# lisqzqng/Video-based-gait-analysis-for-dementia

Measured on AMD Instinct MI355X. Metric: frames/sec (224x224, seq=16), higher is better.
Workload: dtype f32

## Files before the change

### video-based-gait-analysis-for-dementia_amd/csrc/conv_wino4.hip

```cpp
#include "kernels.h"

#include <cstdio>
#include <cstdlib>

namespace grk {

typedef float f32x4 __attribute__((ext_vector_type(4)));
#define GRNET_LDS_AS __attribute__((address_space(3)))

namespace {

#ifdef GRNET_ABLATION
__device__ unsigned long long g_w4phase[8];
#define W4_TICK(var) const unsigned long long var = __builtin_readcyclecounter()
#else
#define W4_TICK(var) do { } while (0)
#endif

constexpr int kCK = 8;
constexpr int kRaw = 6 * 56;
constexpr int kV = 36 * kCK * 16;
constexpr int kMrow = 20;
constexpr size_t kLdsB = sizeof(float) * (2 * kCK * kRaw + 2 * kV);
static_assert(sizeof(float) * 36 * 16 * kMrow <= kLdsB, "the epilogue tile reuses the staging area");

template <typename T>
__device__ __forceinline__ void landed(T& x) { asm volatile("" : "+v"(x)); }

__device__ __forceinline__ void bt_lo(const float* d, float& r0, float& r1, float& r2) {
    const float t1 = fmaf(-4.f, d[2], d[4]), t2 = fmaf(-4.f, d[1], d[3]);
    r0 = fmaf(4.f, d[0], fmaf(-5.f, d[2], d[4]));
    r1 = t1 + t2;
    r2 = t1 - t2;
}
__device__ __forceinline__ void bt_hi(const float* d, float& r3, float& r4, float& r5) {
    const float u1 = d[4] - d[2], u2 = 2.f * (d[3] - d[1]);
    r3 = u1 + u2;
    r4 = u1 - u2;
    r5 = fmaf(4.f, d[1], fmaf(-5.f, d[3], d[5]));
}

template <int NB, int WD, int ABL, bool WSPLIT>
__device__ __forceinline__ void conv_wino4_body(const ConvArgs& a) {
    constexpr bool PAIR = NB == 2 && !WSPLIT;
    constexpr int NLD = PAIR ? 9 : 18;
    constexpr int TPR = WD / 4, TRG = 14 / TPR, kRawW = (4 * TRG + 2) * WD, UPC = kRawW / 4;
    static_assert(WD == 56 || WD == 28, "tile geometry");
    extern __shared__ __align__(16) float smem[];
    float* raw = smem;
    float* V = raw + 2 * kCK * kRaw;
    const int tid = threadIdx.x, lane = tid & 63, wave = tid >> 6, l15 = lane & 15, lq = lane >> 4;

    const int id = a.blk0 + (WSPLIT ? (int)(blockIdx.x >> 1) : (int)blockIdx.x), nb0 = WSPLIT ? 2 * (int)(blockIdx.x & 1) : 0;
    int bx, by;
    if (a.xcd) {
        const int j = id >> 3, x = id & 7, q = j / a.gy;
        by = j - q * a.gy;
        bx = x * (a.gx >> 3) + q;
    } else {
        bx = id / a.gy;
        by = id - bx * a.gy;
    }
    const int groups = ((a.H >> 2) + TRG - 1) / TRG;
    const int img = bx / groups, r = bx - img * groups;
    const int co0 = WSPLIT ? by * 64 : by * (NB * 16);
    constexpr int cstr = WSPLIT ? 4 : NB;
    if (a.prio == 1) __builtin_amdgcn_s_setprio(1);
    else if (a.prio >= 2) __builtin_amdgcn_s_setprio(3);
    const int HW = a.H * a.W;
    const float* inb = a.in + ((size_t)img * a.in_ctot + a.in_coff) * HW;
    const int g0 = (4 * TRG * r - 1) * WD;

    const __amdgpu_buffer_rsrc_t u_rsrc = __builtin_amdgcn_make_buffer_rsrc((void*)a.w, (short)0, 36 * a.CinPad * a.CoutPad * 4, 0x00020000);
    const __amdgpu_buffer_rsrc_t r_rsrc = __builtin_amdgcn_make_buffer_rsrc((void*)inb, (short)0, a.Cin * HW * 4, 0x00020000);
    typedef float bfrag __attribute__((ext_vector_type(PAIR ? 4 : NB)));
    const int nchunks_u = a.CinPad / kCK;
    const int ub = PAIR ? ((lq * a.CoutPad * 2 + co0 * 2 + l15 * 4) * 4 + wave * 9 * nchunks_u * 4 * a.CoutPad * 2 * 4)
                        : ((wave * 9 * a.CinPad + lq) * a.CoutPad + co0 + l15 * cstr + nb0) * 4;
    const int u_point = PAIR ? nchunks_u * 4 * a.CoutPad * 2 * 4 : a.CinPad * a.CoutPad * 4;
    const int u_kstep = 4 * a.CoutPad * 4, u_chunk = PAIR ? 4 * a.CoutPad * 2 * 4 : kCK * a.CoutPad * 4;
    auto load_u = [&](int chunk, int g) -> bfrag {
        const int soff = PAIR ? chunk * u_chunk + g * u_point : chunk * u_chunk + (g >> 1) * u_point + (g & 1) * u_kstep;
        if constexpr (PAIR || NB == 4) return __builtin_bit_cast(bfrag, __builtin_amdgcn_raw_buffer_load_b128(u_rsrc, ub, soff, 0));
        else return __builtin_bit_cast(bfrag, __builtin_amdgcn_raw_buffer_load_b64(u_rsrc, ub, soff, 0));
    };
    int roff[3];
#pragma unroll
    for (int i = 0; i < 3; ++i) {
        const int u = i * 256 + tid, ch = u / UPC, k = u - ch * UPC, gi = g0 + 4 * k;
        const bool unit = u < kCK * UPC, inside = gi >= 0 && gi < HW;
        roff[i] = unit && inside ? (ch * HW + gi) * 4 : -1;
        if (unit && !inside) {
            *reinterpret_cast<f32x4*>(raw + u * 4) = f32x4{0.f, 0.f, 0.f, 0.f};
            *reinterpret_cast<f32x4*>(raw + kCK * kRawW + u * 4) = f32x4{0.f, 0.f, 0.f, 0.f};
        }
    }
    auto issue_raw = [&](int chunk) {
        const int soff = chunk * (kCK * 4) * HW;
        float* dst = raw + (chunk & 1) * (kCK * kRawW);
#pragma unroll
        for (int i = 0; i < 3; ++i)
            if (roff[i] >= 0) __builtin_amdgcn_raw_ptr_buffer_load_lds(r_rsrc, (GRNET_LDS_AS void*)(dst + (i * 256 + wave * 64) * 4), 16, roff[i], soff, 0, 0);
        asm volatile("" ::: "memory");
    };

    const int row16 = tid >> 4, px = tid & 15, chn = row16 & 7;
    const int half = __builtin_amdgcn_readfirstlane(row16 >> 3);
    const int pc = WD == 56 ? px : (px & 7), trl = WD == 56 ? 0 : (px >> 3);
    const bool real = pc < TPR;
    const int rpos = chn * kRawW + (4 * trl) * WD + 4 * (real ? pc : TPR - 1);
    const int slot = real ? trl * TPR + pc : 14 + (WD == 56 ? px - 14 : trl);
    const int vpos = (half * 18) * (kCK * 16) + chn * 16 + slot;
    struct Tf { float d[6][6]; float e[3][6]; };
    auto tf_read = [&](Tf& t, const float* rp) {
#pragma unroll
        for (int i = 0; i < 6; ++i) {
            const f32x4 v = *reinterpret_cast<const f32x4*>(rp + i * WD);
            t.d[i][1] = v[0]; t.d[i][2] = v[1]; t.d[i][3] = v[2]; t.d[i][4] = v[3];
        }
    };
    auto tf_halo = [&](Tf& t) {
#pragma unroll
        for (int i = 0; i < 6; ++i) {
            t.d[i][0] = __int_as_float(__builtin_amdgcn_update_dpp(0, __float_as_int(WD == 56 || real ? t.d[i][4] : 0.f), 0x111, 0xf, 0xf, true));
            t.d[i][5] = __int_as_float(__builtin_amdgcn_update_dpp(0, __float_as_int(real ? t.d[i][1] : 0.f), 0x101, 0xf, 0xf, true));
        }
    };
    auto tf_rows = [&](Tf& t) {
#pragma unroll
        for (int j = 0; j < 6; ++j) {
            const float col[6] = {t.d[0][j], t.d[1][j], t.d[2][j], t.d[3][j], t.d[4][j], t.d[5][j]};
            if (half == 0) bt_lo(col, t.e[0][j], t.e[1][j], t.e[2][j]);
            else bt_hi(col, t.e[0][j], t.e[1][j], t.e[2][j]);
        }
    };
    auto tf_cols = [&](Tf& t, float* vp) {
#pragma unroll
        for (int rr = 0; rr < 3; ++rr) {
            float o[6];
            bt_lo(t.e[rr], o[0], o[1], o[2]);
            bt_hi(t.e[rr], o[3], o[4], o[5]);
#pragma unroll
            for (int c = 0; c < 6; ++c) vp[(rr * 6 + c) * (kCK * 16)] = o[c];
        }
    };

    f32x4 acc[9][NB];
#pragma unroll
    for (int p = 0; p < 9; ++p)
#pragma unroll
        for (int n = 0; n < NB; ++n) acc[p][n] = f32x4{0.f, 0.f, 0.f, 0.f};

    const int nchunks = a.CinPad / kCK;
    bfrag bq[NLD];
    W4_TICK(t_start);
    issue_raw(0);
    if (nchunks > 1) issue_raw(1);
#pragma unroll
    for (int g = 0; g < NLD; ++g) bq[g] = load_u(0, g);
    if constexpr (PAIR) asm volatile("s_waitcnt vmcnt(9)" ::: "memory");
    else asm volatile("s_waitcnt vmcnt(18)" ::: "memory");
    __syncthreads();
    W4_TICK(t_first);
    {
        Tf t;
        tf_read(t, raw + rpos);
        tf_halo(t);
        tf_rows(t);
        tf_cols(t, V + vpos);
    }
    W4_TICK(t_tf0);
    float av[2][6];
    auto load_a = [&](int buf, int c, int set) {
#pragma unroll
        for (int k = 0; k < 6; ++k) {
            const int p = wave * 9 + 3 * c + (k >> 1), ks = k & 1;
            av[set][k] = V[buf * kV + p * (kCK * 16) + (ks * 4 + lq) * 16 + l15];
        }
    };
    auto chunk = [&](int buf, bool with_transform, int next) {
        Tf t;
        const float* rp = raw + (next & 1) * (kCK * kRawW) + rpos;
        float* vp = V + (next & 1) * kV + vpos;
        if (ABL != 3) load_a(buf, 0, 0);
        if (with_transform && ABL != 1 && next + 1 < nchunks) issue_raw(next + 1);
#pragma unroll
        for (int c = 0; c < 3; ++c) {
#pragma unroll
            for (int k = 0; k < 6; ++k) landed(av[c & 1][k]);
            if (with_transform && ABL != 2) {
                if (c == 1) { tf_halo(t); tf_rows(t); }
                if (c == 2) tf_cols(t, vp);
            }
            __builtin_amdgcn_sched_barrier(0);
            if (c < 2 && ABL != 3) load_a(buf, c + 1, (c + 1) & 1);
            if (with_transform && ABL != 1 && c > 0) {
#pragma unroll
                for (int k = 0; k < NLD / 3; ++k) bq[(NLD / 3) * (c - 1) + k] = load_u(next, (NLD / 3) * (c - 1) + k);
            }
            if (with_transform && ABL != 2 && c == 0) tf_read(t, rp);
            __builtin_amdgcn_sched_barrier(0);
#pragma unroll
            for (int k = 0; k < 6; ++k)
#pragma unroll
                for (int n = 0; n < NB; ++n) {
                    const int pi = 3 * c + (k >> 1);
                    const float bfr = PAIR ? bq[pi][(k & 1) * 2 + n] : bq[6 * c + k][n];
                    acc[pi][n] = __builtin_amdgcn_mfma_f32_16x16x4f32(av[c & 1][k], bfr, acc[pi][n], 0, 0, 0);
                }
            __builtin_amdgcn_sched_barrier(0);
        }
        if (with_transform && ABL != 1) {
#pragma unroll
            for (int k = 0; k < NLD / 3; ++k) bq[2 * (NLD / 3) + k] = load_u(next, 2 * (NLD / 3) + k);
        }
    };
    auto meet = [&](bool last) {
        if (last) asm volatile("s_waitcnt vmcnt(0)" ::: "memory");
        else if constexpr (PAIR) asm volatile("s_waitcnt vmcnt(9)" ::: "memory");
        else asm volatile("s_waitcnt vmcnt(18)" ::: "memory");
        __syncthreads();
    };
    for (int ch = 0; ch + 1 < nchunks; ++ch) {
        meet(false);
        chunk(ch & 1, true, ch + 1);
    }
    const bool has_add = a.n_add == 1;
    meet(nchunks > 1);
    const int ec = tid / 14, et = tid - ec * 14, etro = et / TPR, etx = et - etro * TPR, eorow = 4 * (TRG * r + etro);
    const bool ethread = tid < 14 * 16 && eorow < a.H;
    f32x4 radd[4] = {f32x4{0.f, 0.f, 0.f, 0.f}, f32x4{0.f, 0.f, 0.f, 0.f}, f32x4{0.f, 0.f, 0.f, 0.f}, f32x4{0.f, 0.f, 0.f, 0.f}};
    auto fetch_res = [&](int nt) {
        const int co = co0 + (nb0 + nt) * 16 + ec;
        if (has_add && ethread && co < a.Cout) {
            const float* ap = a.add[0] + ((size_t)img * a.add_ctot[0] + a.add_coff[0] + co) * HW + eorow * WD + 4 * etx;
#pragma unroll
            for (int i = 0; i < 4; ++i) radd[i] = *reinterpret_cast<const f32x4*>(ap + i * WD);
        }
    };
    fetch_res(0);
    chunk((nchunks - 1) & 1, false, 0);

    W4_TICK(t_loop);
    float* Mx = smem;
    for (int nt = 0; nt < NB; ++nt) {
        __syncthreads();
#pragma unroll
        for (int pi = 0; pi < 9; ++pi) {
            f32x4 v;
            if constexpr (NB == 4) v = nt == 0 ? acc[pi][0] : nt == 1 ? acc[pi][1] : nt == 2 ? acc[pi][2] : acc[pi][3];
            else v = nt == 0 ? acc[pi][0] : acc[pi][1];
            *reinterpret_cast<f32x4*>(Mx + ((wave * 9 + pi) * 16 + l15) * kMrow + lq * 4) = v;
        }
        __syncthreads();
        const f32x4 rcur[4] = {radd[0], radd[1], radd[2], radd[3]};
        if (nt + 1 < NB) fetch_res(nt + 1);
        if (ethread) {
            const int c = ec, t = et, tx = etx;
            const int co = co0 + (nb0 + nt) * 16 + c, orow = eorow;
            if (co < a.Cout) {
                float s[4][6];
#pragma unroll
                for (int j = 0; j < 6; ++j) {
                    float m[6];
#pragma unroll
                    for (int i = 0; i < 6; ++i) m[i] = Mx[((i * 6 + j) * 16 + c) * kMrow + t];
                    const float p12 = m[1] + m[2], m12 = m[1] - m[2], p34 = m[3] + m[4], m34 = m[3] - m[4];
                    s[0][j] = m[0] + p12 + p34;
                    s[1][j] = fmaf(2.f, m34, m12);
                    s[2][j] = fmaf(4.f, p34, p12);
                    s[3][j] = fmaf(8.f, m34, m12) + m[5];
                }
                const float b = a.bias[co];
                const size_t obase = ((size_t)img * a.out_ctot + a.out_coff + co) * HW + orow * WD + 4 * tx;
#pragma unroll
                for (int i = 0; i < 4; ++i) {
                    const float* q = s[i];
                    const float p12 = q[1] + q[2], m12 = q[1] - q[2], p34 = q[3] + q[4], m34 = q[3] - q[4];
                    f32x4 y = f32x4{q[0] + p12 + p34 + b, fmaf(2.f, m34, m12) + b, fmaf(4.f, p34, p12) + b, fmaf(8.f, m34, m12) + q[5] + b};
                    if (has_add) y += rcur[i];
                    if (a.relu) { y[0] = fmaxf(y[0], 0.f); y[1] = fmaxf(y[1], 0.f); y[2] = fmaxf(y[2], 0.f); y[3] = fmaxf(y[3], 0.f); }
                    *reinterpret_cast<f32x4*>(a.out + obase + i * WD) = y;
                }
            }
        }
    }
#ifdef GRNET_ABLATION
    if ((a.dbg & 8) && tid == 0) {
        W4_TICK(t_end);
        atomicAdd(&g_w4phase[0], t_first - t_start); atomicAdd(&g_w4phase[1], t_tf0 - t_first); atomicAdd(&g_w4phase[2], t_loop - t_tf0);
        atomicAdd(&g_w4phase[3], t_end - t_loop); atomicAdd(&g_w4phase[4], 1ull);
    }
#endif
}

template <int NB, int WD = 56, int ABL = 0, bool WSPLIT = false>
__global__ __launch_bounds__(256) void conv_wino4_f32(const ConvArgs a) { conv_wino4_body<NB, WD, ABL, WSPLIT>(a); }

constexpr int kCKW = 16;
constexpr int kVW = 36 * kCKW * 16;
constexpr size_t kLdsW = sizeof(float) * (2 * kCKW * kRaw + 2 * kVW);
static_assert(sizeof(float) * 2 * 36 * 16 * kMrow <= kLdsW, "the epilogue tiles reuse the staging area");

template <int WD, int NPW>
__device__ __forceinline__ void conv_wino4w_body(const ConvArgs& a) {
    constexpr int TPR = WD / 4, TRG = 14 / TPR, kRawW = (4 * TRG + 2) * WD, UPC = kRawW / 4;
    constexpr int COUTW = 2 * NPW * 16;
    static_assert((WD == 56 || WD == 28) && (NPW == 4 || NPW == 2), "geometry");
    typedef float bfrag __attribute__((ext_vector_type(NPW)));
    extern __shared__ __align__(16) float smem[];
    float* raw = smem;
    float* V = raw + 2 * kCKW * kRaw;
    const int tid = threadIdx.x, lane = tid & 63, wave = __builtin_amdgcn_readfirstlane(tid >> 6), l15 = lane & 15, lq = lane >> 4;
    const int pg = wave & 3, hf = wave >> 2;

    const int id = blockIdx.x;
    int bx, by;
    if (a.xcd) {
        const int j = id >> 3, x = id & 7, q = j / a.gy;
        by = j - q * a.gy;
        bx = x * (a.gx >> 3) + q;
    } else {
        bx = id / a.gy;
        by = id - bx * a.gy;
    }
    const int groups = ((a.H >> 2) + TRG - 1) / TRG;
    const int img = bx / groups, r = bx - img * groups;
    const int co0 = by * COUTW + hf * (NPW * 16);
    const int wpos = NPW == 4 ? co0 : (co0 & ~63) + ((co0 >> 5) & 1) * 2;
    if (a.prio == 1) __builtin_amdgcn_s_setprio(1);
    else if (a.prio >= 2) __builtin_amdgcn_s_setprio(3);
    const int HW = a.H * a.W;
    const float* inb = a.in + ((size_t)img * a.in_ctot + a.in_coff) * HW;
    const int g0 = (4 * TRG * r - 1) * WD;

    const __amdgpu_buffer_rsrc_t u_rsrc = __builtin_amdgcn_make_buffer_rsrc((void*)a.w, (short)0, 36 * a.CinPad * a.CoutPad * 4, 0x00020000);
    const __amdgpu_buffer_rsrc_t r_rsrc = __builtin_amdgcn_make_buffer_rsrc((void*)inb, (short)0, a.Cin * HW * 4, 0x00020000);
    const int ub = ((pg * 9 * a.CinPad + lq) * a.CoutPad + wpos + l15 * 4) * 4;
    const int u_point = a.CinPad * a.CoutPad * 4, u_kstep = 4 * a.CoutPad * 4, u_chunk = kCKW * a.CoutPad * 4;
    auto load_u = [&](int chunk, int q, int e) -> bfrag {
        const int soff = chunk * u_chunk + (3 * (q >> 1) + (e >> 1)) * u_point + (2 * (q & 1) + (e & 1)) * u_kstep;
        if constexpr (NPW == 4) return __builtin_bit_cast(bfrag, __builtin_amdgcn_raw_buffer_load_b128(u_rsrc, ub, soff, 0));
        else return __builtin_bit_cast(bfrag, __builtin_amdgcn_raw_buffer_load_b64(u_rsrc, ub, soff, 0));
    };
    constexpr int NRU = (kCKW * UPC + 511) / 512;
    int roff[NRU];
#pragma unroll
    for (int i = 0; i < NRU; ++i) {
        const int u = i * 512 + tid, ch = u / UPC, k = u - ch * UPC, gi = g0 + 4 * k;
        const bool unit = u < kCKW * UPC, inside = gi >= 0 && gi < HW;
        roff[i] = unit && inside ? (ch * HW + gi) * 4 : -1;
        if (unit && !inside) {
            *reinterpret_cast<f32x4*>(raw + u * 4) = f32x4{0.f, 0.f, 0.f, 0.f};
            *reinterpret_cast<f32x4*>(raw + kCKW * kRawW + u * 4) = f32x4{0.f, 0.f, 0.f, 0.f};
        }
    }
    auto issue_raw = [&](int chunk) {
        const int soff = chunk * (kCKW * 4) * HW;
        float* dst = raw + (chunk & 1) * (kCKW * kRawW);
#pragma unroll
        for (int i = 0; i < NRU; ++i)
            if (roff[i] >= 0) __builtin_amdgcn_raw_ptr_buffer_load_lds(r_rsrc, (GRNET_LDS_AS void*)(dst + (i * 512 + wave * 64) * 4), 16, roff[i], soff, 0, 0);
        asm volatile("" ::: "memory");
    };

    const int row16 = tid >> 4, px = tid & 15, chn = row16 & 15;
    const int pc = WD == 56 ? px : (px & 7), trl = WD == 56 ? 0 : (px >> 3);
    const bool real = pc < TPR;
    const int rpos = chn * kRawW + (4 * trl) * WD + 4 * (real ? pc : TPR - 1);
    const int slot = real ? trl * TPR + pc : 14 + (WD == 56 ? px - 14 : trl);
    const int vpos = (hf * 18) * (kCKW * 16) + chn * 16 + slot;
    auto transform = [&](const float* rp, float* vp) {
        float e[3][6];
        float d[6][6];
#pragma unroll
        for (int i = 0; i < 6; ++i) {
            const f32x4 v = *reinterpret_cast<const f32x4*>(rp + i * WD);
            d[i][1] = v[0]; d[i][2] = v[1]; d[i][3] = v[2]; d[i][4] = v[3];
        }
#pragma unroll
        for (int i = 0; i < 6; ++i) {
            d[i][0] = __int_as_float(__builtin_amdgcn_update_dpp(0, __float_as_int(WD == 56 || real ? d[i][4] : 0.f), 0x111, 0xf, 0xf, true));
            d[i][5] = __int_as_float(__builtin_amdgcn_update_dpp(0, __float_as_int(real ? d[i][1] : 0.f), 0x101, 0xf, 0xf, true));
        }
#pragma unroll
        for (int j = 0; j < 6; ++j) {
            const float col[6] = {d[0][j], d[1][j], d[2][j], d[3][j], d[4][j], d[5][j]};
            if (hf == 0) bt_lo(col, e[0][j], e[1][j], e[2][j]);
            else bt_hi(col, e[0][j], e[1][j], e[2][j]);
        }
#pragma unroll
        for (int rr = 0; rr < 3; ++rr) {
            float o[6];
            bt_lo(e[rr], o[0], o[1], o[2]);
            bt_hi(e[rr], o[3], o[4], o[5]);
#pragma unroll
            for (int c = 0; c < 6; ++c) vp[(rr * 6 + c) * (kCKW * 16)] = o[c];
        }
    };

    f32x4 acc[9][NPW];
#pragma unroll
    for (int p = 0; p < 9; ++p)
#pragma unroll
        for (int n = 0; n < NPW; ++n) acc[p][n] = f32x4{0.f, 0.f, 0.f, 0.f};

    const int nchunks = a.CinPad / kCKW;
    bfrag bq[6];
    float av[2][6];
    auto load_a = [&](int buf, int q, int set) {
#pragma unroll
        for (int e = 0; e < 6; ++e) {
            const int p = pg * 9 + 3 * (q >> 1) + (e >> 1), ks = 2 * (q & 1) + (e & 1);
            av[set][e] = V[buf * kVW + p * (kCKW * 16) + (ks * 4 + lq) * 16 + l15];
        }
    };
    auto multiply = [&](int buf, int ch, bool more) {
        load_a(buf, 0, 0);
#pragma unroll
        for (int q = 0; q < 6; ++q) {
#pragma unroll
            for (int e = 0; e < 6; ++e) landed(av[q & 1][e]);
            __builtin_amdgcn_sched_barrier(0);
            if (q < 5) load_a(buf, q + 1, (q + 1) & 1);
            __builtin_amdgcn_sched_barrier(0);
#pragma unroll
            for (int e = 0; e < 6; ++e) {
                const int pi = 3 * (q >> 1) + (e >> 1);
#pragma unroll
                for (int n = 0; n < NPW; ++n) acc[pi][n] = __builtin_amdgcn_mfma_f32_16x16x4f32(av[q & 1][e], bq[e][n], acc[pi][n], 0, 0, 0);
                __builtin_amdgcn_sched_barrier(0);
                if (q < 5) bq[e] = load_u(ch, q + 1, e);
                else if (more) bq[e] = load_u(ch + 1, 0, e);
                __builtin_amdgcn_sched_barrier(0);
            }
        }
    };

    const bool has_add = a.n_add == 1;
    const int eh = tid >> 8, et2 = tid & 255, ec = et2 / 14, et = et2 - ec * 14, etro = et / TPR, etx = et - etro * TPR, eorow = 4 * (TRG * r + etro);
    const bool ethread = et2 < 14 * 16 && eorow < a.H;
    f32x4 radd[4] = {f32x4{0.f, 0.f, 0.f, 0.f}, f32x4{0.f, 0.f, 0.f, 0.f}, f32x4{0.f, 0.f, 0.f, 0.f}, f32x4{0.f, 0.f, 0.f, 0.f}};
    auto fetch_res = [&](int nt) {
        const int co = by * COUTW + eh * (NPW * 16) + nt * 16 + ec;
        if (has_add && ethread && co < a.Cout) {
            const float* ap = a.add[0] + ((size_t)img * a.add_ctot[0] + a.add_coff[0] + co) * HW + eorow * WD + 4 * etx;
#pragma unroll
            for (int i = 0; i < 4; ++i) radd[i] = *reinterpret_cast<const f32x4*>(ap + i * WD);
        }
    };

    issue_raw(0);
    if (nchunks > 1) issue_raw(1);
#pragma unroll
    for (int e = 0; e < 6; ++e) bq[e] = load_u(0, 0, e);
    asm volatile("s_waitcnt vmcnt(6)" ::: "memory");
    __syncthreads();
    if (hf == 0) transform(raw + rpos, V + vpos);
    for (int k = 0; k < nchunks; ++k) {
        if (hf == 0) {
            asm volatile("s_waitcnt vmcnt(6)" ::: "memory");
            __syncthreads();
            if (k + 2 < nchunks) issue_raw(k + 2);
        }
        const int tk = k + 1 - hf;
        if (tk < nchunks) transform(raw + (tk & 1) * (kCKW * kRawW) + rpos, V + (tk & 1) * kVW + vpos);
        if (hf != 0) {
            asm volatile("s_waitcnt vmcnt(6)" ::: "memory");
            __syncthreads();
            if (k + 2 < nchunks) issue_raw(k + 2);
        }
        if (k + 1 == nchunks) fetch_res(0);
        __builtin_amdgcn_sched_barrier(0);
        multiply(k & 1, k, k + 1 < nchunks);
        __builtin_amdgcn_sched_barrier(0);
    }

    float* Mx = smem + hf * (36 * 16 * kMrow);
    const float* Mr = smem + eh * (36 * 16 * kMrow);
    for (int nt = 0; nt < NPW; ++nt) {
        __syncthreads();
#pragma unroll
        for (int pi = 0; pi < 9; ++pi) {
            f32x4 v;
            if constexpr (NPW == 4) v = nt == 0 ? acc[pi][0] : nt == 1 ? acc[pi][1] : nt == 2 ? acc[pi][2] : acc[pi][3];
            else v = nt == 0 ? acc[pi][0] : acc[pi][1];
            *reinterpret_cast<f32x4*>(Mx + ((pg * 9 + pi) * 16 + l15) * kMrow + lq * 4) = v;
        }
        __syncthreads();
        const f32x4 rcur[4] = {radd[0], radd[1], radd[2], radd[3]};
        if (nt + 1 < NPW) fetch_res(nt + 1);
        if (ethread) {
            const int co = by * COUTW + eh * (NPW * 16) + nt * 16 + ec;
            if (co < a.Cout) {
                float s4[4][6];
#pragma unroll
                for (int j = 0; j < 6; ++j) {
                    float m[6];
#pragma unroll
                    for (int i = 0; i < 6; ++i) m[i] = Mr[((i * 6 + j) * 16 + ec) * kMrow + et];
                    const float p12 = m[1] + m[2], m12 = m[1] - m[2], p34 = m[3] + m[4], m34 = m[3] - m[4];
                    s4[0][j] = m[0] + p12 + p34;
                    s4[1][j] = fmaf(2.f, m34, m12);
                    s4[2][j] = fmaf(4.f, p34, p12);
                    s4[3][j] = fmaf(8.f, m34, m12) + m[5];
                }
                const float b = a.bias[co];
                const size_t obase = ((size_t)img * a.out_ctot + a.out_coff + co) * HW + eorow * WD + 4 * etx;
#pragma unroll
                for (int i = 0; i < 4; ++i) {
                    const float* q = s4[i];
                    const float p12 = q[1] + q[2], m12 = q[1] - q[2], p34 = q[3] + q[4], m34 = q[3] - q[4];
                    f32x4 y = f32x4{q[0] + p12 + p34 + b, fmaf(2.f, m34, m12) + b, fmaf(4.f, p34, p12) + b, fmaf(8.f, m34, m12) + q[5] + b};
                    if (has_add) y += rcur[i];
                    if (a.relu) { y[0] = fmaxf(y[0], 0.f); y[1] = fmaxf(y[1], 0.f); y[2] = fmaxf(y[2], 0.f); y[3] = fmaxf(y[3], 0.f); }
                    *reinterpret_cast<f32x4*>(a.out + obase + i * WD) = y;
                }
            }
        }
    }
}

template <int WD, int NPW>
__global__ __launch_bounds__(512) void conv_wino4w_f32(const ConvArgs a) { conv_wino4w_body<WD, NPW>(a); }

}

int conv_wino4_wide(int cout, int w) {
    static const int wide_env = GRNET_AB(WINO_WIDE, 1);
    if (w == 56) return cout % 128 == 0 ? ((wide_env & 1) ? 4 : 0) : cout == 64 ? ((wide_env & 8) ? 2 : 0) : 0;
    if (w == 28) return cout % 128 == 0 ? ((wide_env & 4) ? 4 : 0) : cout == 64 ? ((wide_env & 2) ? 2 : 0) : 0;
    return 0;
}
int conv_wino4_blocks(int cout, int w) { return (cout % 64 == 0 && !(w == 28 && cout == 64 && !conv_wino4_wide(cout, w))) ? 4 : 2; }

bool conv_wino4_eligible(int cin, int cout, int ks, int stride, int h, int w, int n_add) {
    return ks == 3 && stride == 1 && ((h == 56 && w == 56) || (h == 28 && w == 28)) && n_add <= 1 && cin % kCK == 0 && cout % 32 == 0 && cin >= 32;
}

static size_t wino4_lds() {
    static const size_t pad = (size_t)GRNET_AB(WINO_LDS_PAD, 0);
    return kLdsB + pad;
}

hipError_t conv_wino4_form(const ConvArgs& a, Wino4Form* f) {
    *f = Wino4Form{};
    f->nb = conv_wino4_blocks(a.Cout, a.W);
    if (!conv_wino4_eligible(a.Cin, a.Cout, a.ks, a.stride, a.H, a.W, a.n_add) || a.CinPad % kCK != 0 || a.CoutPad % (f->nb * 16) != 0) return hipErrorInvalidValue;
    if (a.n_add == 1 && a.add_shift[0] != 0) return hipErrorInvalidValue;
    const int npw = conv_wino4_wide(a.Cout, a.W);
    if (npw && a.CinPad % kCKW == 0 && a.CoutPad % (npw * 32) == 0 && !(a.dbg & 32)) {
        const int trg = a.W == 56 ? 1 : 2;
        f->waves = 8;
        f->npw = npw;
        f->gx = a.N * (((a.H >> 2) + trg - 1) / trg);
        f->gy = a.CoutPad / (npw * 32);
        f->xcd = f->gx % 8 == 0 && f->gx >= 16 ? 1 : 0;
        f->full = f->gx * f->gy;
        return hipSuccess;
    }
    const int trg = 14 / (a.W / 4);
    f->waves = 4;
    f->gx = a.N * (((a.H >> 2) + trg - 1) / trg);
    f->gy = a.CoutPad / (f->nb * 16);
    f->xcd = f->gx % 8 == 0 && f->gx >= 16 ? 1 : 0;
    const int total = f->gx * f->gy;
    f->full = total;
    if (f->nb == 2) return hipSuccess;
    static const int split_env = GRNET_AB(WINO_SPLIT, 1);
    int kCUs = 0;
    if (hipError_t e = device_cu_count(&kCUs); e != hipSuccess) return e;
    const int full = total / kCUs * kCUs, rest = total - full;
    if (split_env && full > 0 && rest > 0 && 2 * rest <= kCUs && (!f->xcd || full % 8 == 0)) {
        f->split = 1;
        f->full = full;
        f->rest = rest;
    }
    return hipSuccess;
}

template <int WD>
static hipError_t launch_wino4_w(ConvArgs a, hipStream_t s, const Wino4Form& f, int* n_launches) {
    const size_t kLdsB = wino4_lds();
    a.gx = f.gx;
    a.gy = f.gy;
    a.xcd = f.xcd;
    a.blk0 = 0;
    a.wsplit = 0;
    if (n_launches) *n_launches = 1;
    const int total = a.gx * a.gy;
#ifdef GRNET_ABLATION
    if constexpr (WD == 56) {
        if (a.dbg >= 1 && a.dbg <= 3) {
            auto go = [&](auto kern) { (void)hipFuncSetAttribute(reinterpret_cast<const void*>(kern), hipFuncAttributeMaxDynamicSharedMemorySize, (int)kLdsB); return launch_k(kern, dim3(total), dim3(256), kLdsB, s, a); };
            if (a.dbg == 1) return go(conv_wino4_f32<4, 56, 1>);
            if (a.dbg == 2) return go(conv_wino4_f32<4, 56, 2>);
            return go(conv_wino4_f32<4, 56, 3>);
        }
    }
#endif
    if (f.nb == 2) return launch_k(conv_wino4_f32<2, WD>, dim3(total), dim3(256), kLdsB, s, a);
    if (f.split) {
        hipError_t e = launch_k(conv_wino4_f32<4, WD>, dim3(f.full), dim3(256), kLdsB, s, a);
        if (e != hipSuccess) return e;
        a.blk0 = f.full;
        a.wsplit = 1;
        if (n_launches) *n_launches = 2;
        return launch_k(conv_wino4_f32<2, WD, 0, true>, dim3(2 * f.rest), dim3(256), kLdsB, s, a);
    }
    return launch_k(conv_wino4_f32<4, WD>, dim3(total), dim3(256), kLdsB, s, a);
}

hipError_t launch_conv_wino4(ConvArgs a, hipStream_t s, int* n_launches) {
    static PerDeviceOnce attr;
    int dev = 0;
    if (hipError_t e = current_device(&dev); e != hipSuccess) return e;
    if (hipError_t e = once_per_device(attr, dev, [](int*) {
            hipError_t e = hipSuccess;
            auto set = [&](auto kern) { if (e == hipSuccess) e = hipFuncSetAttribute(reinterpret_cast<const void*>(kern), hipFuncAttributeMaxDynamicSharedMemorySize, (int)wino4_lds()); };
            set(conv_wino4_f32<4, 56>); set(conv_wino4_f32<2, 56>); set(conv_wino4_f32<4, 28>); set(conv_wino4_f32<2, 28>);
            set(conv_wino4_f32<2, 56, 0, true>); set(conv_wino4_f32<2, 28, 0, true>);
            auto setw = [&](auto kern) { if (e == hipSuccess) e = hipFuncSetAttribute(reinterpret_cast<const void*>(kern), hipFuncAttributeMaxDynamicSharedMemorySize, (int)kLdsW); };
            setw(conv_wino4w_f32<56, 4>); setw(conv_wino4w_f32<56, 2>); setw(conv_wino4w_f32<28, 4>); setw(conv_wino4w_f32<28, 2>);
            return e;
        }); e != hipSuccess) return e;
    Wino4Form f;
    if (hipError_t e = conv_wino4_form(a, &f); e != hipSuccess) return e;
    if (f.waves == 8) {
        a.gx = f.gx;
        a.gy = f.gy;
        a.xcd = f.xcd;
        a.blk0 = 0;
        a.wsplit = 0;
        if (n_launches) *n_launches = 1;
        const dim3 grid(a.gx * a.gy);
        if (a.W == 56) return f.npw == 4 ? launch_k(conv_wino4w_f32<56, 4>, grid, dim3(512), kLdsW, s, a) : launch_k(conv_wino4w_f32<56, 2>, grid, dim3(512), kLdsW, s, a);
        return f.npw == 4 ? launch_k(conv_wino4w_f32<28, 4>, grid, dim3(512), kLdsW, s, a) : launch_k(conv_wino4w_f32<28, 2>, grid, dim3(512), kLdsW, s, a);
    }
#ifdef GRNET_ABLATION
    if (GRNET_AB_SET(W4_PHASES)) {
        a.dbg |= 8;
        const hipError_t e = a.W == 56 ? launch_wino4_w<56>(a, s, f, n_launches) : launch_wino4_w<28>(a, s, f, n_launches);
        unsigned long long h[8] = {}, z[8] = {};
        hipStreamSynchronize(s);
        hipMemcpyFromSymbol(h, HIP_SYMBOL(g_w4phase), sizeof(h));
        hipMemcpyToSymbol(HIP_SYMBOL(g_w4phase), z, sizeof(z));
        const double n = h[4] ? (double)h[4] : 1.0;
        fprintf(stderr, "[wino4 phases] %d->%d @%d N%d add %d nb %d wgs %llu: per WG ticks  prologue %.0f  first transform %.0f  chunk loop %.0f (%d chunks)  epilogue %.0f\n",
                a.Cin, a.Cout, a.W, a.N, a.n_add, f.nb, h[4], h[0] / n, h[1] / n, h[2] / n, a.CinPad / kCK, h[3] / n);
        return e;
    }
#endif
    return a.W == 56 ? launch_wino4_w<56>(a, s, f, n_launches) : launch_wino4_w<28>(a, s, f, n_launches);
}

void wino4_transform_filter(const double* g, double* u) {
// ... 36 lines not shown
```

### video-based-gait-analysis-for-dementia_amd/csrc/grnet.cpp

```cpp
#include "../../include/grnet_hip.h"

#include <hip/hip_runtime.h>

#include <cmath>
#include <cstdio>
#include <cstdlib>
#include <algorithm>
#include <cstring>
#include <map>
#include <memory>
#include <string>
#include <tuple>
#include <unordered_map>
#include <vector>

#include "kernels.h"

using namespace grk;

namespace grk { thread_local GraphRecorder* g_recorder = nullptr; }

namespace {

constexpr double kBnEps = 1e-5;
// ... 1084 lines not shown
                } else if (!pinned) {
                    const int pref = from >= 0 ? lane_of[from] : 0;
                    lane = pref;
                    start = std::max(ready, lane_free[pref]);
                    for (int l = 0; l < n_lanes; ++l) {
                        const double st = std::max(ready, lane_free[l]);
                        if (st + hop_us < start) { start = st; lane = l; }
                    }
                }
                if (best < 0 || start < best_start - 1e-9 || (start < best_start + 1e-9 && blevel[i] > blevel[best])) {
                    best = i; best_lane = lane; best_start = start;
                }
            }
            done[best] = 1;
            lane_of[best] = best_lane;
            finish[best] = best_start + est[best];
            lane_free[best_lane] = finish[best];
            for (int u : users[best]) --pending[u];
            order.push_back(best);
        }
        std::vector<Op> out;
        out.reserve(m);
        for (int i : order) {
            Op op = list[i];
            op.lane = lane_of[i];
            op.waits.clear();
            op.record = false;
            out.push_back(std::move(op));
        }
        if (getenv("GRNET_TRACE")) fprintf(stderr, "[grnet] lane schedule: %d ops, estimated makespan %.0f us (sum of estimates %.0f us)\n", m,
                                           *std::max_element(lane_free, lane_free + kLanes), [&] { double t = 0; for (double e : est) t += e; return t; }());
        list.swap(out);
    }

    void analyze_dependencies(std::vector<Op>& ops, std::vector<hipEvent_t>& op_events) {
        std::map<int, std::vector<int>> writers;
        for (int i = 0; i < (int)ops.size(); ++i) {
            Op& op = ops[i];
            for (int buf : op.rd) {
                auto it = writers.find(buf);
                if (it == writers.end()) continue;
                for (int w : it->second)
                    if (ops[w].lane != op.lane) {
                        bool dup = false;
                        for (int x : op.waits) dup |= x == w;
                        if (!dup) op.waits.push_back(w);
                        ops[w].record = true;
                    }
            }
            for (int out : op.wr) writers[out].push_back(i);
        }
        op_events.assign(ops.size(), nullptr);
        if (getenv("GRNET_TRACE")) {
            size_t waits = 0, records = 0;
            for (const Op& op : ops) { waits += op.waits.size(); records += op.record; }
            fprintf(stderr, "[grnet] dependencies: %zu ops, %zu cross-lane waits, %zu recorded events\n", ops.size(), waits, records);
        }
    }

    const HostTensor* find(const std::string& k) const {
        auto it = tensors.find(k);
        return it == tensors.end() ? nullptr : &it->second;
    }

    int upload(const std::vector<float>& h, float** d) {
        int rc = dev_alloc(d, h.size());
        if (rc) return rc;
        if (hipMemcpy(*d, h.data(), h.size() * sizeof(float), hipMemcpyHostToDevice) != hipSuccess)
            return fail(GRNET_EHIP, "hipMemcpy H2D failed");
        return 0;
    }

    int pack_conv(ConvLayer& L) {
        const int cin = L.cin_w, ks = L.ks, taps = ks * ks;
        const int TC = conv_pick_tc(L.cout);
        const bool bf = dtype == 1;
        L.cin_pad = bf ? (L.in.c + L.in2.c + 31) / 32 * 32 : (cin + kConvCK - 1) / kConvCK * kConvCK;
        if (L.in2.c && (!bf || ks != 1 || L.in.c % 32 != 0 || L.segs.size() != 1 || L.seg2.cout != L.cout)) return fail(GRNET_ESTATE, "a two-input launch is a bf16 1x1 convolution with one weight segment per input");
        L.cout_pad = bf ? (L.cout + 31) / 32 * 32 : (L.cout + TC - 1) / TC * TC;
        std::vector<float> wp((size_t)taps * L.cin_pad * L.cout_pad, 0.f), bp(L.cout_pad, 0.f);
        static const int wino4_env = GRNET_AB(WINO4, 2);
        const bool wino4 = !bf && wino4_env && conv_wino4_eligible(L.in.c, L.cout, L.ks, L.stride, L.in.h, L.in.w, (int)L.adds.size()) && L.cin_pad % 8 == 0 &&
                           L.cout_pad % (L.cout % 64 == 0 ? 64 : 32) == 0 && (L.adds.empty() || L.adds[0].shift == 0) &&
                           (L.in.w == 56 || (L.in.c >= 64 && L.cout % 64 == 0));
        const bool wino4s = !bf && wino4_env && cin == L.in.c && conv_wino4s_eligible(L.in.c, L.cout, L.ks, L.stride, L.in.h, L.in.w, (int)L.adds.size()) &&
                            (L.adds.empty() || L.adds[0].shift == 0);
        static const int stem_env = GRNET_AB(STEM, 1);
        const bool stem_shape = cin == L.in.c && L.segs.size() == 1 && conv_stem_eligible(L.in.c, L.cout, L.ks, L.stride, L.in.h, L.in.w, (int)L.adds.size());
        const bool stem = !bf && stem_env && stem_shape, stem_bf = bf && bf16_stem && stem_shape;
        if (bf && bf16_stem && reinterpret_cast<uintptr_t>(L.in.p) == ~(uintptr_t)0 && !stem_bf)
            return fail(GRNET_ESTATE, "bf16 plan without a conversion launch, but its first convolution is not eligible for conv_bf16_stem");
        std::vector<double> wfold(wino4 || wino4s || stem || stem_bf ? (size_t)L.cout * cin * 9 : 0);
        int co0 = 0;
        for (auto& s : L.segs) {
            const HostTensor* w = find(s.wkey);
            if (!w) return fail(GRNET_ENOENT, "missing tensor " + s.wkey);
            if (w->shape.size() != 4 || w->shape[0] != s.cout || w->shape[1] != cin || w->shape[2] != ks || w->shape[3] != ks)
                return fail(GRNET_EINVAL, "bad shape for " + s.wkey);
            std::vector<double> scale(s.cout, 1.0), shift(s.cout, 0.0);
            if (!s.biaskey.empty()) {
                const HostTensor* bt = find(s.biaskey);
                if (!bt || (int)bt->numel() != s.cout) return fail(GRNET_ENOENT, "missing tensor " + s.biaskey);
                for (int c = 0; c < s.cout; ++c) shift[c] = bt->data[c];
            }
            if (!s.bnprefix.empty()) {
                const HostTensor *g = find(s.bnprefix + ".weight"), *be = find(s.bnprefix + ".bias"),
                                 *m = find(s.bnprefix + ".running_mean"), *v = find(s.bnprefix + ".running_var");
                if (!g || !be || !m || !v) return fail(GRNET_ENOENT, "missing BatchNorm tensors " + s.bnprefix + ".*");
                if ((int)g->numel() != s.cout) return fail(GRNET_EINVAL, "bad BatchNorm size " + s.bnprefix);
                for (int c = 0; c < s.cout; ++c) {
                    const double sc = (double)g->data[c] / std::sqrt((double)v->data[c] + kBnEps);
                    shift[c] = (double)be->data[c] + (shift[c] - (double)m->data[c]) * sc;
                    scale[c] = sc;
                }
            }
            for (int co = 0; co < s.cout; ++co) {
                bp[co0 + co] = (float)shift[co];
                for (int ci = 0; ci < cin; ++ci)
                    for (int t = 0; t < taps; ++t) {
                        const double wv = (double)w->data[((size_t)co * cin + ci) * taps + t] * scale[co];
                        wp[bf ? ((((size_t)(ci / 32) * taps + t) * L.cout_pad + co0 + co) * 32 + ci % 32) : ((size_t)t * L.cin_pad + ci) * L.cout_pad + co0 + co] = (float)wv;
                        if (wino4 || wino4s || stem || stem_bf) wfold[((size_t)(co0 + co) * cin + ci) * 9 + t] = wv;
                    }
            }
            co0 += s.cout;
        }
        if (L.in2.c) {
            const ConvSeg& s2 = L.seg2;
            const int cin2 = L.in2.c;
            const HostTensor* w = find(s2.wkey);
            if (!w) return fail(GRNET_ENOENT, "missing tensor " + s2.wkey);
            if (w->shape.size() != 4 || w->shape[0] != s2.cout || w->shape[1] != cin2 || w->shape[2] != 1 || w->shape[3] != 1) return fail(GRNET_EINVAL, "bad shape for " + s2.wkey);
            const HostTensor *g = find(s2.bnprefix + ".weight"), *be = find(s2.bnprefix + ".bias"), *m = find(s2.bnprefix + ".running_mean"), *v = find(s2.bnprefix + ".running_var");
            if (!g || !be || !m || !v) return fail(GRNET_ENOENT, "missing BatchNorm tensors " + s2.bnprefix + ".*");
            if ((int)g->numel() != s2.cout) return fail(GRNET_EINVAL, "bad BatchNorm size " + s2.bnprefix);
            for (int co = 0; co < s2.cout; ++co) {
                const double sc = (double)g->data[co] / std::sqrt((double)v->data[co] + kBnEps);
                bp[co] = (float)((double)bp[co] + (double)be->data[co] - (double)m->data[co] * sc);
                for (int ci = 0; ci < cin2; ++ci) {
                    const int cc = L.in.c + ci;
                    wp[(((size_t)(cc / 32) * taps + 0) * L.cout_pad + co) * 32 + cc % 32] = (float)((double)w->data[(size_t)co * cin2 + ci] * sc);
                }
            }
        }
        int rc;
        if (bf) {
            std::vector<float> packed((wp.size() + 1) / 2, 0.f);
            uint16_t* h16 = reinterpret_cast<uint16_t*>(packed.data());
            for (size_t i = 0; i < wp.size(); ++i) h16[i] = f32_to_bf16(wp[i]);
            if ((rc = upload(packed, &L.w_dev))) return rc;
        } else if ((rc = upload(wp, &L.w_dev))) {
            return rc;
        }
        if ((rc = upload(bp, &L.b_dev))) return rc;
        if (stem) {
            std::vector<float> sw(7 * 4 * 64);
            pack_stem_weights(wfold.data(), sw.data());
            if ((rc = upload(sw, &L.stem_dev))) return rc;
        }
        if (stem_bf) {
            std::vector<float> sw(4 * 64 * 8 / 2);
            pack_stem_weights_bf16(wfold.data(), reinterpret_cast<unsigned short*>(sw.data()));
            if ((rc = upload(sw, &L.stem_dev))) return rc;
        }
        if (wino4s) {
            std::vector<float> uws((size_t)36 * cin * L.cout);
            pack_wino4r_weights(wfold.data(), L.cout, cin, uws.data());
// ... 1896 lines not shown
```

Measured before the change: 4525.

## Pack last row-groups of two 28x28 images into one Winograd block

For 28x28 layers, each image previously took four row-group blocks, the last one only half full (7 tile rows split into groups of two). The new mapping gives each pair of images seven blocks: three full groups per image plus one shared block that computes the final tile row of both images, loading rows from two images into a single staging buffer. This cuts the grid size and the wasted half-empty blocks, at the cost of more complex indexing and a different split heuristic for W=28. It also relaxes the kernel eligibility for input channels down to 16, while the host packing still requires 32.

```diff
diff --git a/video-based-gait-analysis-for-dementia_amd/csrc/conv_wino4.hip b/video-based-gait-analysis-for-dementia_amd/csrc/conv_wino4.hip
--- a/video-based-gait-analysis-for-dementia_amd/csrc/conv_wino4.hip
+++ b/video-based-gait-analysis-for-dementia_amd/csrc/conv_wino4.hip
@@ -39,6 +39,20 @@
     r4 = u1 - u2;
     r5 = fmaf(4.f, d[1], fmaf(-5.f, d[3], d[5]));
 }
+
+struct Group28 { int img, r; bool pair, two; };
+__device__ __forceinline__ Group28 group28(int bx, int n) {
+    const int p = bx / 7, w = bx - 7 * p, i0 = 2 * p;
+    const bool partner = i0 + 1 < n;
+    Group28 g;
+    g.pair = w == 6 || (w == 3 && !partner);
+    g.two = g.pair && partner;
+    g.img = i0 + (w >= 3 && !g.pair ? 1 : 0);
+    g.r = g.pair ? 3 : (w >= 3 ? w - 3 : w);
+    return g;
+}
+constexpr int kPairRows = 6, kPairRow0 = 23;
+constexpr int kPairUPC = kPairRows * 28 / 4;
 
 template <int NB, int WD, int ABL, bool WSPLIT>
 __device__ __forceinline__ void conv_wino4_body(const ConvArgs& a) {
@@ -61,8 +75,11 @@
         bx = id / a.gy;
         by = id - bx * a.gy;
     }
-    const int groups = ((a.H >> 2) + TRG - 1) / TRG;
-    const int img = bx / groups, r = bx - img * groups;
+    int img, r;
+    bool pairg = false, two = false;
+    if constexpr (WD == 56) { img = bx / 14; r = bx - img * 14; }
+    else { const Group28 g = group28(bx, a.N); img = g.img; r = g.r; pairg = g.pair; two = g.two; }
+    const int krw = pairg ? 2 * kPairRows * WD : kRawW;
     const int co0 = WSPLIT ? by * 64 : by * (NB * 16);
     constexpr int cstr = WSPLIT ? 4 : NB;
     if (a.prio == 1) __builtin_amdgcn_s_setprio(1);
@@ -72,7 +89,8 @@
     const int g0 = (4 * TRG * r - 1) * WD;
 
     const __amdgpu_buffer_rsrc_t u_rsrc = __builtin_amdgcn_make_buffer_rsrc((void*)a.w, (short)0, 36 * a.CinPad * a.CoutPad * 4, 0x00020000);
-    const __amdgpu_buffer_rsrc_t r_rsrc = __builtin_amdgcn_make_buffer_rsrc((void*)inb, (short)0, a.Cin * HW * 4, 0x00020000);
+    const int img2 = a.in_ctot * HW * 4;
+    const __amdgpu_buffer_rsrc_t r_rsrc = __builtin_amdgcn_make_buffer_rsrc((void*)inb, (short)0, a.Cin * HW * 4 + (two ? img2 : 0), 0x00020000);
     typedef float bfrag __attribute__((ext_vector_type(PAIR ? 4 : NB)));
     const int nchunks_u = a.CinPad / kCK;
     const int ub = PAIR ? ((lq * a.CoutPad * 2 + co0 * 2 + l15 * 4) * 4 + wave * 9 * nchunks_u * 4 * a.CoutPad * 2 * 4)
@@ -87,17 +105,31 @@
     int roff[3];
 #pragma unroll
     for (int i = 0; i < 3; ++i) {
-        const int u = i * 256 + tid, ch = u / UPC, k = u - ch * UPC, gi = g0 + 4 * k;
-        const bool unit = u < kCK * UPC, inside = gi >= 0 && gi < HW;
-        roff[i] = unit && inside ? (ch * HW + gi) * 4 : -1;
+        const int u = i * 256 + tid;
+        int ch, gi, off2 = 0;
+        bool unit, inside;
+        if (pairg) {
+            ch = u / (2 * kPairUPC);
+            const int k = u - ch * (2 * kPairUPC), lower = k >= kPairUPC ? 1 : 0;
+            gi = kPairRow0 * WD + 4 * (k - lower * kPairUPC);
+            unit = u < kCK * 2 * kPairUPC;
+            inside = gi < HW && (!lower || two);
+            off2 = lower * img2;
+        } else {
+            ch = u / UPC;
+            gi = g0 + 4 * (u - ch * UPC);
+            unit = u < kCK * UPC;
+            inside = gi >= 0 && gi < HW;
+        }
+        roff[i] = unit && inside ? (ch * HW + gi) * 4 + off2 : -1;
         if (unit && !inside) {
             *reinterpret_cast<f32x4*>(raw + u * 4) = f32x4{0.f, 0.f, 0.f, 0.f};
-            *reinterpret_cast<f32x4*>(raw + kCK * kRawW + u * 4) = f32x4{0.f, 0.f, 0.f, 0.f};
+            *reinterpret_cast<f32x4*>(raw + kCK * kRaw + u * 4) = f32x4{0.f, 0.f, 0.f, 0.f};
         }
     }
     auto issue_raw = [&](int chunk) {
         const int soff = chunk * (kCK * 4) * HW;
-        float* dst = raw + (chunk & 1) * (kCK * kRawW);
+        float* dst = raw + (chunk & 1) * (kCK * kRaw);
 #pragma unroll
         for (int i = 0; i < 3; ++i)
             if (roff[i] >= 0) __builtin_amdgcn_raw_ptr_buffer_load_lds(r_rsrc, (GRNET_LDS_AS void*)(dst + (i * 256 + wave * 64) * 4), 16, roff[i], soff, 0, 0);
@@ -108,7 +140,7 @@
     const int half = __builtin_amdgcn_readfirstlane(row16 >> 3);
     const int pc = WD == 56 ? px : (px & 7), trl = WD == 56 ? 0 : (px >> 3);
     const bool real = pc < TPR;
-    const int rpos = chn * kRawW + (4 * trl) * WD + 4 * (real ? pc : TPR - 1);
+    const int rpos = chn * krw + ((pairg ? kPairRows : 4) * trl) * WD + 4 * (real ? pc : TPR - 1);
     const int slot = real ? trl * TPR + pc : 14 + (WD == 56 ? px - 14 : trl);
     const int vpos = (half * 18) * (kCK * 16) + chn * 16 + slot;
     struct Tf { float d[6][6]; float e[3][6]; };
@@ -180,7 +212,7 @@
     };
     auto chunk = [&](int buf, bool with_transform, int next) {
         Tf t;
-        const float* rp = raw + (next & 1) * (kCK * kRawW) + rpos;
+        const float* rp = raw + (next & 1) * (kCK * kRaw) + rpos;
         float* vp = V + (next & 1) * kV + vpos;
         if (ABL != 3) load_a(buf, 0, 0);
         if (with_transform && ABL != 1 && next + 1 < nchunks) issue_raw(next + 1);
@@ -227,13 +259,14 @@
     }
     const bool has_add = a.n_add == 1;
     meet(nchunks > 1);
-    const int ec = tid / 14, et = tid - ec * 14, etro = et / TPR, etx = et - etro * TPR, eorow = 4 * (TRG * r + etro);
-    const bool ethread = tid < 14 * 16 && eorow < a.H;
+    const int ec = tid / 14, et = tid - ec * 14, etro = et / TPR, etx = et - etro * TPR, eorow = 4 * (TRG * r + (pairg ? 0 : etro));
+    const int eimg = img + (pairg ? etro : 0);
+    const bool ethread = tid < 14 * 16 && eimg < a.N;
     f32x4 radd[4] = {f32x4{0.f, 0.f, 0.f, 0.f}, f32x4{0.f, 0.f, 0.f, 0.f}, f32x4{0.f, 0.f, 0.f, 0.f}, f32x4{0.f, 0.f, 0.f, 0.f}};
     auto fetch_res = [&](int nt) {
         const int co = co0 + (nb0 + nt) * 16 + ec;
         if (has_add && ethread && co < a.Cout) {
-            const float* ap = a.add[0] + ((size_t)img * a.add_ctot[0] + a.add_coff[0] + co) * HW + eorow * WD + 4 * etx;
+            const float* ap = a.add[0] + ((size_t)eimg * a.add_ctot[0] + a.add_coff[0] + co) * HW + eorow * WD + 4 * etx;
 #pragma unroll
             for (int i = 0; i < 4; ++i) radd[i] = *reinterpret_cast<const f32x4*>(ap + i * WD);
         }
@@ -272,7 +305,7 @@
                     s[3][j] = fmaf(8.f, m34, m12) + m[5];
                 }
                 const float b = a.bias[co];
-                const size_t obase = ((size_t)img * a.out_ctot + a.out_coff + co) * HW + orow * WD + 4 * tx;
+                const size_t obase = ((size_t)eimg * a.out_ctot + a.out_coff + co) * HW + orow * WD + 4 * tx;
 #pragma unroll
                 for (int i = 0; i < 4; ++i) {
                     const float* q = s[i];
@@ -324,8 +357,11 @@
         bx = id / a.gy;
         by = id - bx * a.gy;
     }
-    const int groups = ((a.H >> 2) + TRG - 1) / TRG;
-    const int img = bx / groups, r = bx - img * groups;
+    int img, r;
+    bool pairg = false, two = false;
+    if constexpr (WD == 56) { img = bx / 14; r = bx - img * 14; }
+    else { const Group28 g = group28(bx, a.N); img = g.img; r = g.r; pairg = g.pair; two = g.two; }
+    const int krw = pairg ? 2 * kPairRows * WD : kRawW;
     const int co0 = by * COUTW + hf * (NPW * 16);
     const int wpos = NPW == 4 ? co0 : (co0 & ~63) + ((co0 >> 5) & 1) * 2;
     if (a.prio == 1) __builtin_amdgcn_s_setprio(1);
@@ -335,7 +371,8 @@
     const int g0 = (4 * TRG * r - 1) * WD;
 
     const __amdgpu_buffer_rsrc_t u_rsrc = __builtin_amdgcn_make_buffer_rsrc((void*)a.w, (short)0, 36 * a.CinPad * a.CoutPad * 4, 0x00020000);
-    const __amdgpu_buffer_rsrc_t r_rsrc = __builtin_amdgcn_make_buffer_rsrc((void*)inb, (short)0, a.Cin * HW * 4, 0x00020000);
+    const int img2 = a.in_ctot * HW * 4;
+    const __amdgpu_buffer_rsrc_t r_rsrc = __builtin_amdgcn_make_buffer_rsrc((void*)inb, (short)0, a.Cin * HW * 4 + (two ? img2 : 0), 0x00020000);
     const int ub = ((pg * 9 * a.CinPad + lq) * a.CoutPad + wpos + l15 * 4) * 4;
     const int u_point = a.CinPad * a.CoutPad * 4, u_kstep = 4 * a.CoutPad * 4, u_chunk = kCKW * a.CoutPad * 4;
     auto load_u = [&](int chunk, int q, int e) -> bfrag {
@@ -343,21 +380,35 @@
         if constexpr (NPW == 4) return __builtin_bit_cast(bfrag, __builtin_amdgcn_raw_buffer_load_b128(u_rsrc, ub, soff, 0));
         else return __builtin_bit_cast(bfrag, __builtin_amdgcn_raw_buffer_load_b64(u_rsrc, ub, soff, 0));
     };
-    constexpr int NRU = (kCKW * UPC + 511) / 512;
+    constexpr int NRU = (kCKW * (WD == 28 ? 2 * kPairUPC : UPC) + 511) / 512;
     int roff[NRU];
 #pragma unroll
     for (int i = 0; i < NRU; ++i) {
-        const int u = i * 512 + tid, ch = u / UPC, k = u - ch * UPC, gi = g0 + 4 * k;
-        const bool unit = u < kCKW * UPC, inside = gi >= 0 && gi < HW;
-        roff[i] = unit && inside ? (ch * HW + gi) * 4 : -1;
+        const int u = i * 512 + tid;
+        int ch, gi, off2 = 0;
+        bool unit, inside;
+        if (pairg) {
+            ch = u / (2 * kPairUPC);
+            const int k = u - ch * (2 * kPairUPC), lower = k >= kPairUPC ? 1 : 0;
+            gi = kPairRow0 * WD + 4 * (k - lower * kPairUPC);
+            unit = u < kCKW * 2 * kPairUPC;
+            inside = gi < HW && (!lower || two);
+            off2 = lower * img2;
+        } else {
+            ch = u / UPC;
+            gi = g0 + 4 * (u - ch * UPC);
+            unit = u < kCKW * UPC;
+            inside = gi >= 0 && gi < HW;
+        }
+        roff[i] = unit && inside ? (ch * HW + gi) * 4 + off2 : -1;
         if (unit && !inside) {
             *reinterpret_cast<f32x4*>(raw + u * 4) = f32x4{0.f, 0.f, 0.f, 0.f};
-            *reinterpret_cast<f32x4*>(raw + kCKW * kRawW + u * 4) = f32x4{0.f, 0.f, 0.f, 0.f};
+            *reinterpret_cast<f32x4*>(raw + kCKW * kRaw + u * 4) = f32x4{0.f, 0.f, 0.f, 0.f};
         }
     }
     auto issue_raw = [&](int chunk) {
         const int soff = chunk * (kCKW * 4) * HW;
-        float* dst = raw + (chunk & 1) * (kCKW * kRawW);
+        float* dst = raw + (chunk & 1) * (kCKW * kRaw);
 #pragma unroll
         for (int i = 0; i < NRU; ++i)
             if (roff[i] >= 0) __builtin_amdgcn_raw_ptr_buffer_load_lds(r_rsrc, (GRNET_LDS_AS void*)(dst + (i * 512 + wave * 64) * 4), 16, roff[i], soff, 0, 0);
@@ -367,7 +418,7 @@
     const int row16 = tid >> 4, px = tid & 15, chn = row16 & 15;
     const int pc = WD == 56 ? px : (px & 7), trl = WD == 56 ? 0 : (px >> 3);
     const bool real = pc < TPR;
-    const int rpos = chn * kRawW + (4 * trl) * WD + 4 * (real ? pc : TPR - 1);
+    const int rpos = chn * krw + ((pairg ? kPairRows : 4) * trl) * WD + 4 * (real ? pc : TPR - 1);
     const int slot = real ? trl * TPR + pc : 14 + (WD == 56 ? px - 14 : trl);
     const int vpos = (hf * 18) * (kCKW * 16) + chn * 16 + slot;
     auto transform = [&](const float* rp, float* vp) {
@@ -438,13 +489,14 @@
     };
 
     const bool has_add = a.n_add == 1;
-    const int eh = tid >> 8, et2 = tid & 255, ec = et2 / 14, et = et2 - ec * 14, etro = et / TPR, etx = et - etro * TPR, eorow = 4 * (TRG * r + etro);
-    const bool ethread = et2 < 14 * 16 && eorow < a.H;
+    const int eh = tid >> 8, et2 = tid & 255, ec = et2 / 14, et = et2 - ec * 14, etro = et / TPR, etx = et - etro * TPR, eorow = 4 * (TRG * r + (pairg ? 0 : etro));
+    const int eimg = img + (pairg ? etro : 0);
+    const bool ethread = et2 < 14 * 16 && eimg < a.N;
     f32x4 radd[4] = {f32x4{0.f, 0.f, 0.f, 0.f}, f32x4{0.f, 0.f, 0.f, 0.f}, f32x4{0.f, 0.f, 0.f, 0.f}, f32x4{0.f, 0.f, 0.f, 0.f}};
     auto fetch_res = [&](int nt) {
         const int co = by * COUTW + eh * (NPW * 16) + nt * 16 + ec;
         if (has_add && ethread && co < a.Cout) {
-            const float* ap = a.add[0] + ((size_t)img * a.add_ctot[0] + a.add_coff[0] + co) * HW + eorow * WD + 4 * etx;
+            const float* ap = a.add[0] + ((size_t)eimg * a.add_ctot[0] + a.add_coff[0] + co) * HW + eorow * WD + 4 * etx;
 #pragma unroll
             for (int i = 0; i < 4; ++i) radd[i] = *reinterpret_cast<const f32x4*>(ap + i * WD);
         }
@@ -464,7 +516,7 @@
             if (k + 2 < nchunks) issue_raw(k + 2);
         }
         const int tk = k + 1 - hf;
-        if (tk < nchunks) transform(raw + (tk & 1) * (kCKW * kRawW) + rpos, V + (tk & 1) * kVW + vpos);
+        if (tk < nchunks) transform(raw + (tk & 1) * (kCKW * kRaw) + rpos, V + (tk & 1) * kVW + vpos);
         if (hf != 0) {
             asm volatile("s_waitcnt vmcnt(6)" ::: "memory");
             __syncthreads();
@@ -506,7 +558,7 @@
                     s4[3][j] = fmaf(8.f, m34, m12) + m[5];
                 }
                 const float b = a.bias[co];
-                const size_t obase = ((size_t)img * a.out_ctot + a.out_coff + co) * HW + eorow * WD + 4 * etx;
+                const size_t obase = ((size_t)eimg * a.out_ctot + a.out_coff + co) * HW + eorow * WD + 4 * etx;
 #pragma unroll
                 for (int i = 0; i < 4; ++i) {
                     const float* q = s4[i];
@@ -535,33 +587,34 @@
 int conv_wino4_blocks(int cout, int w) { return (cout % 64 == 0 && !(w == 28 && cout == 64 && !conv_wino4_wide(cout, w))) ? 4 : 2; }
 
 bool conv_wino4_eligible(int cin, int cout, int ks, int stride, int h, int w, int n_add) {
-    return ks == 3 && stride == 1 && ((h == 56 && w == 56) || (h == 28 && w == 28)) && n_add <= 1 && cin % kCK == 0 && cout % 32 == 0 && cin >= 32;
+    return ks == 3 && stride == 1 && ((h == 56 && w == 56) || (h == 28 && w == 28)) && n_add <= 1 && cin % kCK == 0 && cout % 32 == 0 && cin >= 16;
 }
 
 static size_t wino4_lds() {
     static const size_t pad = (size_t)GRNET_AB(WINO_LDS_PAD, 0);
     return kLdsB + pad;
 }
+
+static int wino4_groups(int n, int w) { return w == 56 ? 14 * n : 7 * (n / 2) + 4 * (n & 1); }
 
 hipError_t conv_wino4_form(const ConvArgs& a, Wino4Form* f) {
     *f = Wino4Form{};
     f->nb = conv_wino4_blocks(a.Cout, a.W);
     if (!conv_wino4_eligible(a.Cin, a.Cout, a.ks, a.stride, a.H, a.W, a.n_add) || a.CinPad % kCK != 0 || a.CoutPad % (f->nb * 16) != 0) return hipErrorInvalidValue;
+    if (a.CinPad != a.Cin) return hipErrorInvalidValue;
     if (a.n_add == 1 && a.add_shift[0] != 0) return hipErrorInvalidValue;
     const int npw = conv_wino4_wide(a.Cout, a.W);
     if (npw && a.CinPad % kCKW == 0 && a.CoutPad % (npw * 32) == 0 && !(a.dbg & 32)) {
-        const int trg = a.W == 56 ? 1 : 2;
         f->waves = 8;
         f->npw = npw;
-        f->gx = a.N * (((a.H >> 2) + trg - 1) / trg);
+        f->gx = wino4_groups(a.N, a.W);
         f->gy = a.CoutPad / (npw * 32);
         f->xcd = f->gx % 8 == 0 && f->gx >= 16 ? 1 : 0;
         f->full = f->gx * f->gy;
         return hipSuccess;
     }
-    const int trg = 14 / (a.W / 4);
     f->waves = 4;
-    f->gx = a.N * (((a.H >> 2) + trg - 1) / trg);
+    f->gx = wino4_groups(a.N, a.W);
     f->gy = a.CoutPad / (f->nb * 16);
     f->xcd = f->gx % 8 == 0 && f->gx >= 16 ? 1 : 0;
     const int total = f->gx * f->gy;
@@ -570,8 +623,12 @@
     static const int split_env = GRNET_AB(WINO_SPLIT, 1);
     int kCUs = 0;
     if (hipError_t e = device_cu_count(&kCUs); e != hipSuccess) return e;
+    if (a.W == 28) {
+        const int gx4 = 4 * a.N, total4 = gx4 * f->gy, full4 = total4 / kCUs * kCUs, rest4 = total4 - full4, xcd4 = gx4 % 8 == 0 && gx4 >= 16;
+        if (!(full4 > 0 && rest4 > 0 && 2 * rest4 <= kCUs && (!xcd4 || full4 % 8 == 0))) return hipSuccess;
+    }
     const int full = total / kCUs * kCUs, rest = total - full;
-    if (split_env && full > 0 && rest > 0 && 2 * rest <= kCUs && (!f->xcd || full % 8 == 0)) {
+    if (split_env && full > 0 && rest > 0 && (a.W == 28 || 2 * rest <= kCUs) && (!f->xcd || full % 8 == 0)) {
         f->split = 1;
         f->full = full;
         f->rest = rest;
diff --git a/video-based-gait-analysis-for-dementia_amd/csrc/grnet.cpp b/video-based-gait-analysis-for-dementia_amd/csrc/grnet.cpp
--- a/video-based-gait-analysis-for-dementia_amd/csrc/grnet.cpp
+++ b/video-based-gait-analysis-for-dementia_amd/csrc/grnet.cpp
@@ -1190,7 +1190,7 @@
         static const int wino4_env = GRNET_AB(WINO4, 2);
         const bool wino4 = !bf && wino4_env && conv_wino4_eligible(L.in.c, L.cout, L.ks, L.stride, L.in.h, L.in.w, (int)L.adds.size()) && L.cin_pad % 8 == 0 &&
                            L.cout_pad % (L.cout % 64 == 0 ? 64 : 32) == 0 && (L.adds.empty() || L.adds[0].shift == 0) &&
-                           (L.in.w == 56 || (L.in.c >= 64 && L.cout % 64 == 0));
+                           L.in.c >= 32 && (L.in.w == 56 || (L.in.c >= 64 && L.cout % 64 == 0));
         const bool wino4s = !bf && wino4_env && cin == L.in.c && conv_wino4s_eligible(L.in.c, L.cout, L.ks, L.stride, L.in.h, L.in.w, (int)L.adds.size()) &&
                             (L.adds.empty() || L.adds[0].shift == 0);
         static const int stem_env = GRNET_AB(STEM, 1);
```

Measured after the change: 4548 (median of 6 runs). No clear change (+0.5%).
